# gabrevaya/LatentDiffEq.jl

Hardware: AMD Instinct MI355X
Metric: trajectories/sec (fwd+adjoint) GOKU pendulum, batch=256, 1/2/4/8 GPU (higher is better)
Workload: dtype f32; 1 GPU; goku_pendulum: GOKU pendulum D=2 P=1 T=50 Tsit5 abstol=1e-6 reltol=1e-3, per-trajectory; batch_per_gpu=256, global_batch=256, save_points=50, rccl_ranks=1, parallelism=dp1 (batch sharded by trajectory, no data-path collective), submission=hipGraph replays of ≤ 256 captured steps (each step = lde_forward + lde_adjoint)

## Files before the change

### latentdiffeq.jl_amd/csrc/lde_pend_lp.h

```cpp
#pragma once

namespace lp {
struct Tab {
  double C[8];
  double Ab[8][8];
  double Et[8];
  double RA[3][8];
  double RR[8][3];
  double A[8][8], BT[8];
};
constexpr Tab make_tab() {
  Tab t{};
  constexpr double a[8][8] = {
      {0, 0, 0, 0, 0, 0, 0, 0},
      {0, 0, 0, 0, 0, 0, 0, 0},
      {0, 0.161, 0, 0, 0, 0, 0, 0},
      {0, -0.008480655492356989, 0.335480655492357, 0, 0, 0, 0, 0},
      {0, 2.8971530571054935, -6.359448489975075, 4.3622954328695815, 0, 0, 0, 0},
      {0, 5.325864828439257, -11.748883564062828, 7.4955393428898365, -0.09249506636175525, 0, 0, 0},
      {0, 5.86145544294642, -12.92096931784711, 8.159367898576159, -0.071584973281401, -0.028269050394068383, 0, 0},
      {0, 0.09646076681806523, 0.01, 0.4798896504144996, 1.379008574103742, -3.290069515436081, 2.324710524099774, 0}};
  constexpr double bt[8] = {0, -0.00178001105222577714, -0.0008164344596567469, 0.007880878010261995, -0.1447110071732629,
                            0.5823571654525552, -0.45808210592918697, 0.015151515151515152};
  constexpr double rr[8][3] = {{0, 0, 0},
                               {-2.763706197274826, 2.9132554618219126, -1.0530884977290216},
                               {0.13169999999999998, -0.2234, 0.1017},
                               {3.9302962368947516, -5.941033872131505, 2.490627285651253},
                               {-12.411077166933676, 30.33818863028232, -16.548102889244902},
                               {37.50931341651104, -88.1789048947664, 47.37952196281928},
                               {-27.896526289197286, 65.09189467479366, -34.87065786149661},
                               {1.5, -4.0, 2.5}};
  for (int i = 0; i < 8; i++) {
    t.BT[i] = bt[i];
    double c = 0;
    for (int j = 0; j < 8; j++) { t.A[i][j] = a[i][j]; c += a[i][j]; }
    t.C[i] = c;
    for (int m = 0; m < 3; m++) t.RR[i][m] = rr[i][m];
  }
  for (int i = 0; i < 8; i++)
    for (int l = 0; l < 8; l++) {
      double s = 0;
      for (int j = 0; j < 8; j++) s += a[i][j] * a[j][l];
      t.Ab[i][l] = s;
    }
  for (int l = 0; l < 8; l++) {
    double s = 0;
    for (int j = 0; j < 8; j++) s += bt[j] * a[j][l];
    t.Et[l] = s;
    for (int m = 0; m < 3; m++) {
      double q = 0;
      for (int j = 0; j < 8; j++) q += rr[j][m] * a[j][l];
      t.RA[m][l] = q;
    }
  }
  return t;
}
constexpr Tab TB = make_tab();
static_assert(TB.Ab[2][1] == 0 && TB.Ab[3][2] == 0 && TB.Ab[4][3] == 0 && TB.Ab[5][4] == 0 && TB.Ab[6][5] == 0 && TB.Ab[7][6] == 0, "Nyström structure");
static_assert(TB.C[6] > 0.999999999 && TB.C[6] < 1.000000001 && TB.C[7] > 0.999999999 && TB.C[7] < 1.000000001, "c₆ = c₇ = 1");

constexpr int COPIES = 16;
constexpr int RECF = 12;
constexpr int STEPF = COPIES * RECF;

template <int CTRL>
__device__ __forceinline__ float dpp(float v) {
  return __int_as_float(__builtin_amdgcn_update_dpp(0, __float_as_int(v), CTRL, 0xf, 0xf, true));
}
constexpr float TWO_PI = 6.283185307179586f;
#ifndef LDE_LP_SIN
#define LDE_LP_SIN 0
#endif
__device__ __forceinline__ float sin_turns(float t) { return LDE_LP_SIN ? fast_sin(t * TWO_PI) : __builtin_amdgcn_sinf(t); }
constexpr int SWAP = 0xB1;
constexpr int EVEN = 0xA0;
constexpr int ODD = 0xF5;
}

#if LDE_PEND_PROF
#define LPPROF(i) do { if (blockIdx.x == 0 && (threadIdx.x & 63) == 0) { g_pprof[2 * (i)] = wall_clock64(); g_pprof[2 * (i) + 1] = __builtin_readcyclecounter(); } } while (0)
#define LPPROF_VAL(i, v) do { if (blockIdx.x == 0 && (threadIdx.x & 63) == 0) g_pprof[i] = (v); } while (0)
#else
#define LPPROF(i) do { } while (0)
#define LPPROF_VAL(i, v) do { } while (0)
#endif
template <int NH>
struct LpShape {
  static constexpr int LP_NH = NH;
  static constexpr int LP_SW = NH >= 4 ? 2 : 0;
};
template <bool REC, int NH = 4>
__global__ void __launch_bounds__(64 * (1 + NH)) k_pend_forward_lp(const float2* __restrict__ z0, const float* __restrict__ theta,
                                                         const double* __restrict__ ts_g, KOpts o,
                                                         float2* __restrict__ z_out, int32_t* __restrict__ retcode,
                                                         int32_t* __restrict__ st_nfe, int32_t* __restrict__ st_nacc,
                                                         int32_t* __restrict__ st_nrej, int32_t* __restrict__ st_ret) {
  using namespace lp;
  constexpr int LP_NH = LpShape<NH>::LP_NH, LP_SW = LpShape<NH>::LP_SW;
  __shared__ __attribute__((aligned(16))) float s_rec[SH_CAP * STEPF];
  __shared__ int s_cnt[64];
  __shared__ int s_fin;
  __shared__ int s_fail;
  const int T = o.T, B = o.B, tid = threadIdx.x, lane = tid & 63, w = tid >> 6;
  const int chunk = gridDim.x >> 3;
  const int b = (blockIdx.x & 7) * chunk + (blockIdx.x >> 3);
  const bool valid = b < B;
  const int bc = valid ? b : B - 1;
  const double t_first = o.t_first, tend = o.t_last;
  const float o_abstol = o.abstol, o_reltol = o.reltol, o_beta1 = o.beta1, o_beta2 = o.beta2, o_inv_gamma = o.inv_gamma, o_q_lo = o.q_lo,
              o_q_hi = o.q_hi, o_qmin = o.qmin;
  const double o_dtmin = o.dtmin, o_dt_fixed = o.dt_fixed;
  const long long o_maxiters = o.maxiters;
  const int rec_cap = o.rec.cap;
  int32_t* const rec_n = o.rec.n;
  double *const rec_t = o.rec.t, *const rec_dt = o.rec.dt;
  float2* const rec_y = reinterpret_cast<float2*>(o.rec.y);
  asm volatile("" ::"s"(o_abstol), "s"(o_reltol), "s"(o_beta1), "s"(o_beta2), "s"(o_inv_gamma), "s"(o_q_lo), "s"(o_q_hi), "s"(o_qmin), "s"(o_dtmin),
               "s"(o_dt_fixed), "s"(o_maxiters), "s"(T), "s"(B), "s"(chunk), "s"(t_first), "s"(tend), "s"(z0), "s"(theta), "s"(ts_g), "s"(z_out),
               "s"(retcode), "s"(st_nfe), "s"(st_nacc), "s"(st_nrej), "s"(st_ret));
  if (REC) asm volatile("" ::"s"(rec_cap), "s"(rec_n), "s"(rec_t), "s"(rec_dt), "s"(rec_y));
  const float2 zi = z0[bc];
  PendFwd<0> f(theta[bc]);
  const float ngl = f.ngl;
  if (tid < 64) s_cnt[tid] = 0;
  if (tid == 0) { s_fin = 0; s_fail = 0; }
  __syncthreads();
  constexpr int NS = 6;
  float* const myrec = s_rec + (lane >> 2) * RECF;

  if (w == LP_SW) {
    LPPROF(8);
    const bool ev = (lane & 1) == 0;
    auto sel = [&](double a, double c) -> float { return ev ? (float)a : (float)c; };
    const float K11 = sel(TB.Ab[3][1], 0.0);
    const float GK11 = K11 * (ngl * INV_2PI);
    const f32x2 C12 = {sel(TB.C[3], TB.C[2]), sel(TB.C[5], TB.C[4])};
    const f32x2 KP1 = {sel(TB.Ab[5][1], TB.Ab[4][1]), sel(TB.Ab[7][1], TB.Ab[6][1])};
    const f32x2 KPo1 = {sel(TB.Ab[5][3], TB.Ab[4][2]), sel(TB.Ab[7][3], TB.Ab[6][2])};
    const f32x2 KPp1 = {sel(TB.Ab[5][2], 0.0), sel(TB.Ab[7][2], TB.Ab[6][3])};
    const float K3o2 = sel(TB.Ab[7][5], TB.Ab[6][4]), K3p2 = sel(TB.Ab[7][4], 0.0);
    const f32x2 Q1 = {sel(TB.Ab[7][1], TB.A[7][1]), sel(TB.Et[1], TB.BT[1])};
    const f32x2 Qo1 = {sel(TB.Ab[7][3], TB.A[7][2]), sel(TB.Et[3], TB.BT[2])}, Qp1 = {sel(TB.Ab[7][2], TB.A[7][3]), sel(TB.Et[2], TB.BT[3])};
    const f32x2 Qo2 = {sel(TB.Ab[7][5], TB.A[7][4]), sel(TB.Et[5], TB.BT[4])}, Qp2 = {sel(TB.Ab[7][4], TB.A[7][5]), sel(TB.Et[4], TB.BT[5])};
    const f32x2 Qo3 = {sel(0.0, TB.A[7][6]), sel(0.0, TB.BT[6])};
    const float Ep3 = sel(TB.Et[6], TB.BT[7]);
    const float evm = ev ? 1.f : 0.f;
    const float glt = ngl * INV_2PI;
    const float ca = 0.5f * o_beta1, cb = 0.5f * o_beta2, c0 = 0.5f * (o_beta1 - o_beta2) - log2f(o_inv_gamma);
    const float iq_lo = o_qmin, iq_hi = 1.0f / o_q_lo;
    float abst = o_abstol * INV_2PI, relt = o_reltol;
    asm volatile("" : "+v"(abst), "+v"(relt));

    int ret = LDE_RET_SUCCESS, nfe = 0, nacc = 0, nrej = 0;
    double t = t_first;
    float dt = 0.f;
    constexpr float LQ_MIN = -13.287712379549449f;
    constexpr float LG_MIN = 2.0f * LQ_MIN + 1.0f;
    float lgold = LG_MIN;
    const int maxit = o_maxiters > 0x7fffffffLL ? 0x7fffffff : (int)o_maxiters;
    const float dtmin = (float)o_dtmin;
    if (valid && lane == 0) z_out[b] = zi;
    const double dtmax_d = tend - t;
    const float dtmax = (float)dtmax_d;
    float s1 = hw_sin(zi.x, turn_anchor(zi.x));
    nfe = 1;
    if (o_dt_fixed > 0) dt = (float)fmin(o_dt_fixed, dtmax_d);
    else {
      f.anchor(zi.x);
      const float ya[2] = {zi.x, zi.y}, fa[2] = {zi.y, ngl * s1};
      dt = (float)init_dt<2>(f, ya, fa, 1.0f, dtmax_d, o);
      nfe++;
    }
    float yc = (ev ? zi.x : zi.y) * INV_2PI;
    bool active = __any(t < tend) && maxit > 0;
    if (__any(t < tend) && !active) ret = LDE_RET_MAXITERS;
    LPPROF(9);
    float rem = (float)(tend - t);
    bool last = __any(dt >= rem * 0.99999988f);
    float h = last ? rem : dt;
    for (;;) {
      int n = 0;
      float* rp = myrec + (lane & 1) * 4;
      const double t_round = t;
      const float xr = dpp<EVEN>(yc), vr = dpp<ODD>(yc);
      int lim = min(SH_CAP, maxit - (nacc + nrej));
      bool go = active && lim > 0;
      while (go) {
        float xa = dpp<EVEN>(yc);
        const float wa = dpp<ODD>(yc);
        asm volatile("" : "+v"(xa));
        const float xi0 = xa - rintf(xa);
        const float hw = h * wa, hg = h * glt, hhg = hg * h;
        const float scale = ev ? hhg : hg;
        const f32x2 A12 = C12 * f32x2{hw, hw} + f32x2{xi0, xi0};
        f32x2 P = KP1 * f32x2{s1, s1}, Q = Q1 * f32x2{s1, s1};
        const float g1 = sin_turns(fmaf(h, fmaf(h, GK11 * s1, C12.x * wa), xi0));
        const float p1 = dpp<SWAP>(g1);
        P = KPo1 * f32x2{g1, g1} + P;
        P = KPp1 * f32x2{p1, p1} + P;
        const float g2 = sin_turns(fmaf(hhg, P.x, A12.y));
        const float p2 = dpp<SWAP>(g2);
        float in3 = fmaf(K3o2, g2, P.y);
        in3 = fmaf(K3p2, p2, in3);
        const float g3 = sin_turns(fmaf(hhg, in3, xi0 + hw));
        const float p3 = dpp<SWAP>(g3);
        Q = Qo1 * f32x2{g1, g1} + Q;
        Q = Qp1 * f32x2{p1, p1} + Q;
        Q = Qo2 * f32x2{g2, g2} + Q;
        Q = Qp2 * f32x2{p2, p2} + Q;
        Q = Qo3 * f32x2{g3, g3} + Q;
        const float newc = fmaf(scale, Q.x, fmaf(evm, hw, yc));
        const float rs = fast_rcp(fmaf(max_abs(yc, newc), relt, abst));
        const float r = (scale * fmaf(Ep3, p3, Q.y)) * rs;
        float r2 = r * r;
        asm volatile("" : "+v"(r2));
        const float m2 = r2 + dpp<SWAP>(r2);
        const float mq = fmaf(0.f, newc, m2);
        const bool ok = !__any(!(mq <= 2.0f));
        const float lg = __builtin_amdgcn_logf(m2);
        const float iq = __builtin_amdgcn_fmed3f(__builtin_amdgcn_exp2f(fmaf(-ca, lg, fmaf(cb, lgold, c0))), iq_lo, iq_hi);
        const float dtn = h * iq;
        const double t_n = t + (double)h;
        const float rem_n = (float)(tend - t_n), remc_n = rem_n * 0.99999988f;
        asm volatile("" :: "v"(dtn), "v"(remc_n));
        if (__builtin_expect(!ok, 0)) {
          const bool fin = !__any(!(fabsf(newc) < __builtin_inff()));
          nrej++;
          lim--;
          if (!fin) {
            if (__any(h > dtmin)) dt = h * o_qmin;
            else { ret = LDE_RET_NONFINITE; active = false; nrej--; }
          } else {
            dt = h * fast_rcp(fminf(o_q_hi, __builtin_amdgcn_exp2f(o_beta1 * fmaf(0.5f, lg, -0.5f)) * o_inv_gamma));
            if (__any(dt < dtmin)) { ret = LDE_RET_DTMIN; active = false; }
          }
          last = __any(dt >= rem * 0.99999988f);
          h = last ? rem : dt;
          if (!active || n >= lim) go = false;
          continue;
        }
        {
          *reinterpret_cast<f32x4*>(rp) = f32x4{g1, g2, g3, newc};
          myrec[n * STEPF + 8 + (lane & 1)] = h;
          rp += STEPF;
          n++;
          asm volatile("" ::: "memory");
          __hip_atomic_store(&s_cnt[lane], n, __ATOMIC_RELAXED, __HIP_MEMORY_SCOPE_WORKGROUP);
          yc = newc;
          s1 = dpp<EVEN>(g3);
          t = t_n;
          rem = rem_n;
          dt = dtn;
          lgold = max_f(lg, LG_MIN);
          active = !last;
          if (last || n >= lim) go = false;
          h = dtn >= remc_n ? rem_n : dtn;
          last = __any(dtn >= remc_n);
        }
      }
      nacc += n;
      LPPROF(10);
      LPPROF_VAL(30, nacc + nrej);
      if (active && nacc + nrej >= maxit) { ret = LDE_RET_MAXITERS; active = false; }
      if (ret != LDE_RET_SUCCESS && lane == 0) __hip_atomic_store(&s_fail, 1, __ATOMIC_RELAXED, __HIP_MEMORY_SCOPE_WORKGROUP);
      asm volatile("" ::: "memory");
      if (lane == 0) __hip_atomic_store(&s_fin, active ? 1 : 2, __ATOMIC_RELAXED, __HIP_MEMORY_SCOPE_WORKGROUP);
      if (REC) {
        const int i0 = nacc - n;
        const bool mine = lane < n;
        const float* ri = s_rec + (size_t)(mine ? lane : 0) * STEPF;
        const float* rq = s_rec + (size_t)(mine && lane > 0 ? lane - 1 : 0) * STEPF;
        const float hi = ri[8];
        const float2 ys = lane == 0 ? (i0 == 0 ? zi : make_float2(xr * TWO_PI, vr * TWO_PI)) : make_float2(rq[3] * TWO_PI, rq[7] * TWO_PI);
        double tacc = t_round, ti = t_round;
        const int hbits = __float_as_int(hi);
        for (int i = 0; i < n; i++) {
          if (lane == i) ti = tacc;
          tacc += (double)__int_as_float(__builtin_amdgcn_readlane(hbits, i));
        }
        if (valid && mine && i0 + lane < rec_cap) {
          rec_t[(size_t)(i0 + lane) * B + b] = ti;
          rec_dt[(size_t)(i0 + lane) * B + b] = (double)hi;
          rec_y[(size_t)(i0 + lane) * B + b] = ys;
        }
      }
      if (!active) break;
      __syncthreads();
      s_cnt[lane] = 0;
      if (lane == 0) s_fin = 0;
      __syncthreads();
    }
    if (ret != LDE_RET_SUCCESS) {
      __syncthreads();
      if (valid) {
        const float qn = __int_as_float(0x7fc00000);
        for (int j = lane; j < T; j += 64) z_out[(size_t)j * B + b] = make_float2(qn, qn);
      }
    }
    if (valid && lane == 0) {
      if (retcode) retcode[b] = ret;
      st_ret[b] = ret;
      st_nfe[b] = nfe + NS * (nacc + nrej);
      st_nacc[b] = nacc;
      st_nrej[b] = nrej;
      if (REC) rec_n[b] = ret == LDE_RET_SUCCESS ? nacc : 0;
    }
    LPPROF(11);
    return;
  }

  const int hid = w < LP_SW ? w : w - 1;
#if LDE_PEND_PROF
  long long pq[12] = {0, 0, 0, 0, 0, 0, 0, 0, 0, 0, 0, 0};
  const long long pq_in = __builtin_readcyclecounter();
#endif
  const double dinf = __longlong_as_double(0x7ff0000000000000LL);
  int jq = 1 + lane;
  double tj = jq < T ? ts_g[jq] : dinf;
  double tn = t_first;
  f32x2 ys = {zi.x, zi.y};
  float sg1 = hw_sin(zi.x, turn_anchor(zi.x));
  int nrec0 = 0;
  auto advance = [&](int from, int to) {
    for (int q = from; q < to; q++) {
      const float hq = myrec[(size_t)q * STEPF + 8];
      tn = (hq == (float)(tend - tn)) ? tend : tn + (double)hq;
    }
    if (to > from) {
      const float* rl = myrec + (size_t)(to - 1) * STEPF;
      ys = f32x2{rl[3], rl[7]} * TWO_PI;
      sg1 = rl[2];
    }
  };
  for (;;) {
    int n2 = 0, fin;
    for (;;) {
      const int m = n2 + (hid + LP_NH - (nrec0 + n2) % LP_NH) % LP_NH;
      fin = __hip_atomic_load(&s_fin, __ATOMIC_RELAXED, __HIP_MEMORY_SCOPE_WORKGROUP);
      const int cnt = __hip_atomic_load(&s_cnt[lane], __ATOMIC_RELAXED, __HIP_MEMORY_SCOPE_WORKGROUP);
      asm volatile("" ::: "memory");
      if (m < cnt) {
#if LDE_PEND_PROF
        const long long pc0 = __builtin_readcyclecounter();
#endif
        advance(n2, m);
#if LDE_PEND_PROF
        asm volatile("" : "+v"(ys), "+v"(sg1));
        const long long pc1 = __builtin_readcyclecounter();
#endif
        const float* rc = myrec + (size_t)m * STEPF;
        const f32x4 qe = *reinterpret_cast<const f32x4*>(rc), qo = *reinterpret_cast<const f32x4*>(rc + 4);
        const float h = rc[8];
        const f32x2 ye = f32x2{qe[3], qo[3]} * TWO_PI;
        const double t1 = (h == (float)(tend - tn)) ? tend : tn + (double)h;
        while (tj <= tn) {
          jq += 64;
          tj = jq < T ? ts_g[jq] : dinf;
        }
#if LDE_PEND_PROF
        const long long pc2 = __builtin_readcyclecounter();
        long long pc3 = pc2;
#endif
        if (__any(tj <= t1)) {
          f32x2 k0 = {0.f, 0.f}, P2 = {0.f, 0.f}, P3 = {0.f, 0.f}, P4 = {0.f, 0.f};
          float rh = 0.f;
          if (__any(tj < t1)) {
            rh = fast_rcp(h);
            const float sg[8] = {0.f, sg1, qo[0], qe[0], qo[1], qe[1], qo[2], qe[2]};
            const float hg = h * ngl;
            float px[3], pv[3];
#pragma unroll
            for (int mm = 0; mm < 3; mm++) {
              float ax = (float)TB.RA[mm][1] * sg[1], av = (float)TB.RR[1][mm] * sg[1];
#pragma unroll
              for (int l = 2; l <= 6; l++) ax = fmaf((float)TB.RA[mm][l], sg[l], ax);
#pragma unroll
              for (int j = 2; j <= 7; j++) av = fmaf((float)TB.RR[j][mm], sg[j], av);
              px[mm] = hg * ax;
              pv[mm] = ngl * av;
            }
            k0 = f32x2{ys.y, ngl * sg1};
            P2 = f32x2{px[0], pv[0]};
            P3 = f32x2{px[1], pv[1]};
            P4 = f32x2{px[2], pv[2]};
          }
#if LDE_PEND_PROF
          asm volatile("" : "+v"(P2), "+v"(P3), "+v"(P4));
          pc3 = __builtin_readcyclecounter();
#endif
          while (tj <= t1) {
            float2 out;
            if (tj >= t1) out = make_float2(ye.x, ye.y);
            else {
              const float th = (float)(tj - tn) * rh;
              out.x = tsit5_dense_eval<2>(th, h, ys.x, k0.x, P2.x, P3.x, P4.x);
              out.y = tsit5_dense_eval<2>(th, h, ys.y, k0.y, P2.y, P3.y, P4.y);
            }
            if (valid) z_out[(size_t)jq * B + b] = out;
            jq += 64;
            tj = jq < T ? ts_g[jq] : dinf;
          }
        }
        tn = t1;
        ys = ye;
        sg1 = qe[2];
        n2 = m + 1;
#if LDE_PEND_PROF
        { const long long pc4 = __builtin_readcyclecounter(); pq[0] += pc4 - pc0; pq[1] += 1; pq[7] += pc1 - pc0; pq[8] += pc2 - pc1; pq[9] += pc3 - pc2; pq[10] += pc4 - pc3; }
#endif
        continue;
      }
#if LDE_PEND_PROF
      pq[4] += 1;
#endif
      if (fin) {
        advance(n2, cnt);
        n2 = cnt;
        break;
      }
    }
    nrec0 += n2;
    if (fin == 2) break;
    __syncthreads();
    __syncthreads();
  }
#if LDE_PEND_PROF
  if (blockIdx.x == 0 && hid == 0 && lane == 0) {
    for (int i = 0; i < 5; i++) g_pprof[i] = pq[i];
    for (int i = 7; i < 11; i++) g_pprof[i] = pq[i];
    g_pprof[6] = __builtin_readcyclecounter() - pq_in;
  }
  if (blockIdx.x == 0 && lane == 0 && hid < 3) { g_pprof[2 * (12 + hid)] = wall_clock64(); g_pprof[2 * (12 + hid) + 1] = __builtin_readcyclecounter(); }
#endif
  if (__hip_atomic_load(&s_fail, __ATOMIC_RELAXED, __HIP_MEMORY_SCOPE_WORKGROUP)) {
    asm volatile("s_waitcnt vmcnt(0)" ::: "memory");
    __syncthreads();
  }
}
```

Measured before the change: 24.97 million trajectories/s.

## Move final-step dense output and recording off the helper waves onto solver wave

The dense-output interpolation is factored into a direction-templated helper. For the last accepted step, the solver wave now writes the remaining save points itself, walking backward from the end. In the final round, trajectory recording is moved from the solver wave to the helper waves, which track per-lane step start times. This is meant to shorten the critical tail, since helpers no longer have to interpolate the final step after the solver finishes. It adds ablation hooks (LDE_PEND_ABL with a global launch counter) and more complex bookkeeping conditions that carry a correctness risk.

Result: slower. 24.72 million trajectories/s (-1.0%).

```diff
diff --git a/latentdiffeq.jl_amd/csrc/lde_pend_lp.h b/latentdiffeq.jl_amd/csrc/lde_pend_lp.h
--- a/latentdiffeq.jl_amd/csrc/lde_pend_lp.h
+++ b/latentdiffeq.jl_amd/csrc/lde_pend_lp.h
@@ -84,6 +84,55 @@
 #define LPPROF(i) do { } while (0)
 #define LPPROF_VAL(i, v) do { } while (0)
 #endif
+#if LDE_PEND_ABL == 6 || LDE_PEND_ABL == 7
+static __device__ int g_lp_abl_launches;
+#endif
+template <int DIR>
+__device__ __forceinline__ void lp_dense_step(const double tn, const double t1, const float h, const f32x2 ys, const f32x2 ye, const float sg1,
+                                              const f32x4 qe, const f32x4 qo, const float ngl, const double* __restrict__ ts_g, const int T,
+                                              int& jq, double& tj, float2* __restrict__ z_out, const int B, const int b, const bool valid,
+                                              long long& prof_mid) {
+  using namespace lp;
+  const double dinf = __longlong_as_double(0x7ff0000000000000LL);
+  f32x2 k0 = {0.f, 0.f}, P2 = {0.f, 0.f}, P3 = {0.f, 0.f}, P4 = {0.f, 0.f};
+  float rh = 0.f;
+  if (__any(DIR > 0 ? tj < t1 : (tj > tn && tj < t1))) {
+    rh = fast_rcp(h);
+    const float sg[8] = {0.f, sg1, qo[0], qe[0], qo[1], qe[1], qo[2], qe[2]};
+    const float hg = h * ngl;
+    float px[3], pv[3];
+#pragma unroll
+    for (int mm = 0; mm < 3; mm++) {
+      float ax = (float)TB.RA[mm][1] * sg[1], av = (float)TB.RR[1][mm] * sg[1];
+#pragma unroll
+      for (int l = 2; l <= 6; l++) ax = fmaf((float)TB.RA[mm][l], sg[l], ax);
+#pragma unroll
+      for (int j = 2; j <= 7; j++) av = fmaf((float)TB.RR[j][mm], sg[j], av);
+      px[mm] = hg * ax;
+      pv[mm] = ngl * av;
+    }
+    k0 = f32x2{ys.y, ngl * sg1};
+    P2 = f32x2{px[0], pv[0]};
+    P3 = f32x2{px[1], pv[1]};
+    P4 = f32x2{px[2], pv[2]};
+  }
+#if LDE_PEND_PROF
+  asm volatile("" : "+v"(P2), "+v"(P3), "+v"(P4));
+  prof_mid = __builtin_readcyclecounter();
+#endif
+  while (DIR > 0 ? tj <= t1 : tj > tn) {
+    float2 out;
+    if (tj >= t1) out = make_float2(ye.x, ye.y);
+    else {
+      const float th = (float)(tj - tn) * rh;
+      out.x = tsit5_dense_eval<2>(th, h, ys.x, k0.x, P2.x, P3.x, P4.x);
+      out.y = tsit5_dense_eval<2>(th, h, ys.y, k0.y, P2.y, P3.y, P4.y);
+    }
+    if (valid) z_out[(size_t)jq * B + b] = out;
+    jq += DIR;
+    tj = DIR > 0 ? (jq < T ? ts_g[jq] : dinf) : (jq >= 1 ? ts_g[jq] : -dinf);
+  }
+}
 template <int NH>
 struct LpShape {
   static constexpr int LP_NH = NH;
@@ -122,9 +171,20 @@
   const float2 zi = z0[bc];
   PendFwd<0> f(theta[bc]);
   const float ngl = f.ngl;
+  int jf = T - 1 - lane;
+  double tjf = jf >= 1 ? ts_g[jf] : -__longlong_as_double(0x7ff0000000000000LL);
+#if LDE_PEND_ABL == 6 || LDE_PEND_ABL == 7
+  int abl_n = g_lp_abl_launches;
+#endif
   if (tid < 64) s_cnt[tid] = 0;
   if (tid == 0) { s_fin = 0; s_fail = 0; }
   __syncthreads();
+#if LDE_PEND_ABL == 6 || LDE_PEND_ABL == 7
+  asm volatile("" : "+v"(abl_n));
+  const bool abl_skip = __builtin_amdgcn_readfirstlane(abl_n) >= (LDE_PEND_ABL == 6 ? 4 : 0x7fffffff);
+#else
+  constexpr bool abl_skip = false;
+#endif
   constexpr int NS = 6;
   float* const myrec = s_rec + (lane >> 2) * RECF;
 
@@ -152,7 +212,7 @@
     asm volatile("" : "+v"(abst), "+v"(relt));
 
     int ret = LDE_RET_SUCCESS, nfe = 0, nacc = 0, nrej = 0;
-    double t = t_first;
+    double t = t_first, t0 = t_first;
     float dt = 0.f;
     constexpr float LQ_MIN = -13.287712379549449f;
     constexpr float LG_MIN = 2.0f * LQ_MIN + 1.0f;
@@ -178,14 +238,16 @@
     float rem = (float)(tend - t);
     bool last = __any(dt >= rem * 0.99999988f);
     float h = last ? rem : dt;
+    int n = 0;
     for (;;) {
-      int n = 0;
+      n = 0;
       float* rp = myrec + (lane & 1) * 4;
       const double t_round = t;
       const float xr = dpp<EVEN>(yc), vr = dpp<ODD>(yc);
       int lim = min(SH_CAP, maxit - (nacc + nrej));
       bool go = active && lim > 0;
       while (go) {
+        t0 = t;
         float xa = dpp<EVEN>(yc);
         const float wa = dpp<ODD>(yc);
         asm volatile("" : "+v"(xa));
@@ -265,13 +327,14 @@
       if (ret != LDE_RET_SUCCESS && lane == 0) __hip_atomic_store(&s_fail, 1, __ATOMIC_RELAXED, __HIP_MEMORY_SCOPE_WORKGROUP);
       asm volatile("" ::: "memory");
       if (lane == 0) __hip_atomic_store(&s_fin, active ? 1 : 2, __ATOMIC_RELAXED, __HIP_MEMORY_SCOPE_WORKGROUP);
-      if (REC) {
+      if (REC && (active || ret != LDE_RET_SUCCESS || (n == 1 && nacc > 1))) {
         const int i0 = nacc - n;
         const bool mine = lane < n;
         const float* ri = s_rec + (size_t)(mine ? lane : 0) * STEPF;
         const float* rq = s_rec + (size_t)(mine && lane > 0 ? lane - 1 : 0) * STEPF;
         const float hi = ri[8];
         const float2 ys = lane == 0 ? (i0 == 0 ? zi : make_float2(xr * TWO_PI, vr * TWO_PI)) : make_float2(rq[3] * TWO_PI, rq[7] * TWO_PI);
+        asm volatile("" ::"v"(hi));
         double tacc = t_round, ti = t_round;
         const int hbits = __float_as_int(hi);
         for (int i = 0; i < n; i++) {
@@ -290,6 +353,21 @@
       if (lane == 0) s_fin = 0;
       __syncthreads();
     }
+    if (ret == LDE_RET_SUCCESS && n > 0 && !(n == 1 && nacc > 1) && !abl_skip) {
+      const float* rc = myrec + (size_t)(n - 1) * STEPF;
+      const float* rl = myrec + (size_t)(n >= 2 ? n - 2 : 0) * STEPF;
+      const f32x4 qe = *reinterpret_cast<const f32x4*>(rc), qo = *reinterpret_cast<const f32x4*>(rc + 4);
+      const float hf = rc[8];
+      f32x2 ysf = f32x2{rl[3], rl[7]} * TWO_PI, yef = f32x2{qe[3], qo[3]} * TWO_PI;
+      float sgf = rl[2];
+      if (n < 2) {
+        ysf = f32x2{zi.x, zi.y};
+        sgf = hw_sin(zi.x, turn_anchor(zi.x));
+      }
+      asm volatile("" : "+v"(ysf), "+v"(yef));
+      long long unused;
+      lp_dense_step<-64>(t0, tend, hf, ysf, yef, sgf, qe, qo, ngl, ts_g, T, jf, tjf, z_out, B, b, valid, unused);
+    }
     if (ret != LDE_RET_SUCCESS) {
       __syncthreads();
       if (valid) {
@@ -305,6 +383,9 @@
       st_nrej[b] = nrej;
       if (REC) rec_n[b] = ret == LDE_RET_SUCCESS ? nacc : 0;
     }
+#if LDE_PEND_ABL == 6 || LDE_PEND_ABL == 7
+    if (blockIdx.x == 0 && lane == 0) atomicAdd(&g_lp_abl_launches, 1);
+#endif
     LPPROF(11);
     return;
   }
@@ -321,9 +402,12 @@
   f32x2 ys = {zi.x, zi.y};
   float sg1 = hw_sin(zi.x, turn_anchor(zi.x));
   int nrec0 = 0;
+  double ts_l = t_first;
+  f32x2 ys_r = ys;
   auto advance = [&](int from, int to) {
     for (int q = from; q < to; q++) {
       const float hq = myrec[(size_t)q * STEPF + 8];
+      if (REC) ts_l = lane == q ? tn : ts_l;
       tn = (hq == (float)(tend - tn)) ? tend : tn + (double)hq;
     }
     if (to > from) {
@@ -353,6 +437,7 @@
         const float h = rc[8];
         const f32x2 ye = f32x2{qe[3], qo[3]} * TWO_PI;
         const double t1 = (h == (float)(tend - tn)) ? tend : tn + (double)h;
+        if (REC) ts_l = lane == m ? tn : ts_l;
         while (tj <= tn) {
           jq += 64;
           tj = jq < T ? ts_g[jq] : dinf;
@@ -361,45 +446,26 @@
         const long long pc2 = __builtin_readcyclecounter();
         long long pc3 = pc2;
 #endif
-        if (__any(tj <= t1)) {
-          f32x2 k0 = {0.f, 0.f}, P2 = {0.f, 0.f}, P3 = {0.f, 0.f}, P4 = {0.f, 0.f};
-          float rh = 0.f;
-          if (__any(tj < t1)) {
-            rh = fast_rcp(h);
-            const float sg[8] = {0.f, sg1, qo[0], qe[0], qo[1], qe[1], qo[2], qe[2]};
-            const float hg = h * ngl;
-            float px[3], pv[3];
-#pragma unroll
-            for (int mm = 0; mm < 3; mm++) {
-              float ax = (float)TB.RA[mm][1] * sg[1], av = (float)TB.RR[1][mm] * sg[1];
-#pragma unroll
-              for (int l = 2; l <= 6; l++) ax = fmaf((float)TB.RA[mm][l], sg[l], ax);
-#pragma unroll
-              for (int j = 2; j <= 7; j++) av = fmaf((float)TB.RR[j][mm], sg[j], av);
-              px[mm] = hg * ax;
-              pv[mm] = ngl * av;
+        if (t1 == tend && !(m == 0 && nrec0 > 0)) {
+          if (REC && !abl_skip) {
+            const bool mine = lane <= m;
+            const float* ri = s_rec + (size_t)(mine ? lane : 0) * STEPF;
+            const float* rq = s_rec + (size_t)(mine && lane > 0 ? lane - 1 : 0) * STEPF;
+            const float hi = ri[8];
+            const float2 y0r = lane == 0 ? make_float2(ys_r.x, ys_r.y) : make_float2(rq[3] * TWO_PI, rq[7] * TWO_PI);
+            if (valid && mine && nrec0 + lane < rec_cap) {
+              rec_t[(size_t)(nrec0 + lane) * B + b] = ts_l;
+              rec_dt[(size_t)(nrec0 + lane) * B + b] = (double)hi;
+              rec_y[(size_t)(nrec0 + lane) * B + b] = y0r;
             }
-            k0 = f32x2{ys.y, ngl * sg1};
-            P2 = f32x2{px[0], pv[0]};
-            P3 = f32x2{px[1], pv[1]};
-            P4 = f32x2{px[2], pv[2]};
           }
-#if LDE_PEND_PROF
-          asm volatile("" : "+v"(P2), "+v"(P3), "+v"(P4));
-          pc3 = __builtin_readcyclecounter();
-#endif
-          while (tj <= t1) {
-            float2 out;
-            if (tj >= t1) out = make_float2(ye.x, ye.y);
-            else {
-              const float th = (float)(tj - tn) * rh;
-              out.x = tsit5_dense_eval<2>(th, h, ys.x, k0.x, P2.x, P3.x, P4.x);
-              out.y = tsit5_dense_eval<2>(th, h, ys.y, k0.y, P2.y, P3.y, P4.y);
-            }
-            if (valid) z_out[(size_t)jq * B + b] = out;
-            jq += 64;
-            tj = jq < T ? ts_g[jq] : dinf;
-          }
+        } else if (__any(tj <= t1)) {
+#if LDE_PEND_PROF
+          lp_dense_step<64>(tn, t1, h, ys, ye, sg1, qe, qo, ngl, ts_g, T, jq, tj, z_out, B, b, valid, pc3);
+#else
+          long long unused;
+          lp_dense_step<64>(tn, t1, h, ys, ye, sg1, qe, qo, ngl, ts_g, T, jq, tj, z_out, B, b, valid, unused);
+#endif
         }
         tn = t1;
         ys = ye;
@@ -423,6 +489,7 @@
     if (fin == 2) break;
     __syncthreads();
     __syncthreads();
+    ys_r = ys;
   }
 #if LDE_PEND_PROF
   if (blockIdx.x == 0 && hid == 0 && lane == 0) {
```
